# pedroand6/Voxel-Raytracer

Measured on AMD Instinct MI355X. Metric: Mrays/s at 1920×1080 primary rays; achieved HBM GB/s vs peak, higher is better.
Workload: dtype f32

## Files before the change

### voxel-raytracer_amd/__init__.py

```python
import ctypes as C
import os
import subprocess

import numpy as np

HERE = os.path.dirname(os.path.abspath(__file__))
CSRC = os.path.join(HERE, "csrc")
HIP_LIB = os.environ.get("VRT_HIP_LIB") or os.path.join(HERE, "libvrt_hip.so")
HOST_LIB = os.path.join(HERE, "libvrt_host.so")
TEST_LIB = os.path.join(HERE, "libvrt_hip_test.so")
OPT_RAY_TABLES, OPT_EMPTY_OCTANTS, OPT_DISPLAY_KERNEL, OPT_FULL_OPAQUE, OPT_HEAVY_TILES, OPT_MISS_TILES = 1, 2, 3, 4, 5, 6

MODE_PRIMARY, MODE_PRIMARY_SHADOW, MODE_FULL = 0, 1, 2
MODES = {"primary": MODE_PRIMARY, "primary_shadow": MODE_PRIMARY_SHADOW, "full": MODE_FULL}
ACCUM_JITTER = 1


class VrtError(RuntimeError):
    pass


def build(targets=("../libvrt_hip.so", "../libvrt_hip_test.so", "../libvrt_host.so")):
    subprocess.check_call(["make", "-j8", "-C", CSRC, *targets])

# ... 491 lines not shown

def miss_mask(texels, inv_proj, inv_view, cam_pos, width, height, voxel_scale=1.0, world_min=(-1023, -1023, -1023),
              world_max=(1024, 1024, 1024)):
    L = test_lib()
    L.vrt_test_miss_mask.argtypes = [C.c_void_p, C.c_size_t, C.POINTER(C.c_int32), C.POINTER(C.c_int32), C.c_float,
                                     C.POINTER(C.c_float), C.POINTER(C.c_float), C.POINTER(C.c_float), C.c_int, C.c_int,
                                     C.c_void_p, C.POINTER(C.c_int32)]
    t = np.ascontiguousarray(texels, np.uint8)
    ip = np.ascontiguousarray(inv_proj, np.float32).reshape(-1)
    iv = np.ascontiguousarray(inv_view, np.float32).reshape(-1)
    cp = np.zeros(4, np.float32)
    cp[:len(cam_pos)] = np.asarray(cam_pos, np.float32).reshape(-1)[:4]
    mask = np.zeros(((height + 7) // 8, (width + 7) // 8), np.uint8)
    stats = (C.c_int32 * 2)()
    r = L.vrt_test_miss_mask(t.ctypes.data if t.size else None, t.size, (C.c_int32 * 3)(*world_min), (C.c_int32 * 3)(*world_max),
                             float(voxel_scale), _fptr(ip), _fptr(iv), _fptr(cp), int(width), int(height), mask.ctypes.data, stats)
    if r < 0:
        raise VrtError(f"vrt_test_miss_mask failed ({r})")
    if r == 0:
        return None
    return mask, int(stats[0]), bool(stats[1])


def test_tile_order(tile_ticks, wave_slots, device=0):
    L = test_lib()
    t = np.ascontiguousarray(tile_ticks, np.uint32).reshape(-1)
    assert t.size % 4 == 0
    n = t.size // 4
    L.vrt_test_tile_order.argtypes = [C.c_int, C.c_void_p, C.c_uint32, C.c_uint32, C.c_void_p, C.c_void_p]
    order = np.zeros(n, np.uint32)
    split = np.zeros(1, np.uint32)
    r = L.vrt_test_tile_order(device, t.ctypes.data, n, wave_slots, order.ctypes.data, split.ctypes.data)
    if r:
        raise VrtError(f"vrt_test_tile_order failed ({r})")
    return order, int(split[0])



def tree_is_opaque(texels):
    L = test_lib()
    L.vrt_test_tree_is_opaque.argtypes = [C.c_void_p, C.c_size_t]
    t = np.ascontiguousarray(texels, np.uint8)
    r = L.vrt_test_tree_is_opaque(t.ctypes.data if t.size else None, t.size)
    if r < 0:
        raise VrtError(f"vrt_test_tree_is_opaque failed ({r})")
    return r == 1
# ... 484 lines not shown
```

### voxel-raytracer_amd/csrc/vrt_args.h

```cpp
#pragma once
#include <hip/hip_runtime.h>
#include <stdint.h>

namespace vrt {

struct F3 { float x, y, z; };
struct I3 { int x, y, z; };

constexpr int kMaxViews = 4;
constexpr int kGroupTiles = 4;
constexpr int kSplitParts = 8, kSplitMaxGroups = 64;
struct View {
    float inv_proj[16];
    float inv_view[16];
    float cam_pos[4];
    uint32_t *out_rgba;
    int2 *out_id;
    uint32_t eye0, eye1;
    uint32_t first_w0, first_w1, first_node, first_anode;
    int first_s, first_as, first_valid;
    const float *gen_x, *gen_y;
    float gen_z;
    uint32_t gen_fast;
    const uint8_t *miss;
    uint32_t miss_stamp;
};

struct ViewSet {
    View v[kMaxViews];
};

struct KArgs {
    int n_views;
    float voxel_scale;
    int wmin[3];
    int wmax[3];
    float global_light[4];
    float light_dir[3];
    float light_inv[3], light_push[3], light_dposf[3];
    int light_dpos[3];
    int shade_fast;
    int highlighted[3];
    int tex_dim;
    int width, height;
    int row0, n_rows, tile_rows, row_stride;
    int compact;
    uint32_t tiles_x_magic;
    int row_mode;
// ... 24 lines not shown
```

### voxel-raytracer_amd/csrc/vrt_common.hip.h

```cpp
#pragma once

#include "vrt_args.h"

namespace vrt {

#define VRT_DEV __device__ __forceinline__

VRT_DEV float fmin_c(float a, float b) { return b < a ? b : a; }
VRT_DEV float fmax_c(float a, float b) { return a < b ? b : a; }
VRT_DEV float dot3(F3 a, F3 b) { return (a.x * b.x + a.y * b.y) + a.z * b.z; }
VRT_DEV float len3(F3 a) { return __builtin_sqrtf(dot3(a, a)); }
VRT_DEV F3 scale3(F3 a, float s) { return F3{a.x * s, a.y * s, a.z * s}; }
VRT_DEV F3 add3(F3 a, F3 b) { return F3{a.x + b.x, a.y + b.y, a.z + b.z}; }
VRT_DEV F3 sub3(F3 a, F3 b) { return F3{a.x - b.x, a.y - b.y, a.z - b.z}; }
VRT_DEV F3 normalize3(F3 a) { return scale3(a, 1.0f / __builtin_sqrtf(dot3(a, a))); }

VRT_DEV float rcp_inrange(float x) {
    float y = __builtin_amdgcn_rcpf(x);
    y = __builtin_fmaf(__builtin_fmaf(-x, y, 1.0f), y, y);
    const float q = __builtin_fmaf(__builtin_fmaf(-x, y, 1.0f), y, y);
    return __builtin_fmaf(__builtin_fmaf(-x, q, 1.0f), y, q);
}
VRT_DEV float sqrt_inrange(float x) {
    const float s = __builtin_amdgcn_sqrtf(x);
// ... 106 lines not shown
    asm volatile("" : "+s"(p));
    return (LateView)p;
}

struct LateOut {
    uint32_t *out_rgba;
    int2 *out_id;
    int width, compact;
};
VRT_DEV LateOut late_out(LateArgs la, LateView lv) { return LateOut{lv->out_rgba, lv->out_id, la->width, la->compact}; }

VRT_DEV F3 shader_ray_dir(const KArgs &a, const View &vw, float fx, float fy) {
    float u = (fx / (float)a.width) * 2.0f - 1.0f;
    float v = (fy / (float)a.height) * 2.0f - 1.0f;
    float view[4];
    mat_vec(vw.inv_proj, u, v, -1.0f, 1.0f, view);
    if (__builtin_fabsf(view[3]) > 1e-6f) { float w = view[3]; view[0] = view[0] / w; view[1] = view[1] / w; view[2] = view[2] / w; view[3] = view[3] / w; }
    F3 vd = normalize3(F3{view[0], view[1], view[2]});
    float wd4[4];
    mat_vec(vw.inv_view, vd.x, vd.y, vd.z, 0.0f, wd4);
    return normalize3(F3{wd4[0], wd4[1], wd4[2]});
}

VRT_DEV F3 primary_ray_dir(const KArgs &a, const View &vw, int px, int py) {
    if (vw.gen_fast) {
        const F3 vd = normalize3_inrange(F3{vw.gen_x[px], vw.gen_y[py], vw.gen_z});
        float wd4[4];
        mat_vec(vw.inv_view, vd.x, vd.y, vd.z, 0.0f, wd4);
        const F3 d = normalize3_inrange(F3{wd4[0], wd4[1], wd4[2]});
        return scale3(d, rcp_inrange(sqrt_inrange(dot3(d, d))));
    }
    const F3 d = shader_ray_dir(a, vw, (float)px, (float)py);
    return scale3(d, 1.0f / __builtin_sqrtf(dot3(d, d)));
}

VRT_DEV float jitter_x(uint32_t k) { return (float)(__builtin_bitreverse32(k) >> 8) * 0x1p-24f; }
VRT_DEV float jitter_y(uint32_t k) {
    uint32_t y = 0u, v = 1u << 31;
    for (uint32_t i = k; i; i >>= 1, v ^= v >> 1)
        if (i & 1u) y ^= v;
    return (float)(y >> 8) * 0x1p-24f;
}

VRT_DEV F3 jittered_ray_dir(const KArgs &a, const View &vw, int px, int py, uint32_t sample) {
    const float fx = (float)px + jitter_x(sample), fy = (float)py + jitter_y(sample);
    const F3 d = shader_ray_dir(a, vw, fx, fy);
    return scale3(d, 1.0f / __builtin_sqrtf(dot3(d, d)));
}

struct LensRay { F3 o, dir; uint32_t eye0, eye1; };
VRT_DEV LensRay lens_ray(const KArgs &a, const View &vw, int px, int py, float jx, float jy, float aperture, float focus, float lx, float ly) {
    const float fx = (float)px + jx, fy = (float)py + jy;
    const F3 d = shader_ray_dir(a, vw, fx, fy);
    const F3 e{vw.cam_pos[0], vw.cam_pos[1], vw.cam_pos[2]};
    LensRay r;
    r.o = e; r.dir = d; r.eye0 = r.eye1 = 0u;
    const F3 R{vw.inv_view[0], vw.inv_view[1], vw.inv_view[2]}, U{vw.inv_view[4], vw.inv_view[5], vw.inv_view[6]},
             Z{vw.inv_view[8], vw.inv_view[9], vw.inv_view[10]};
    const float cosd = -dot3(d, Z);
    if (!(aperture == 0.0f || (lx == 0.0f && ly == 0.0f) || !(cosd > 0.0f))) {
        const float sx = aperture * lx, sy = aperture * ly;
        r.o = add3(add3(e, scale3(R, sx)), scale3(U, sy));
        const float t = focus / cosd;
        const F3 p = add3(e, scale3(d, t));
        r.dir = normalize3(sub3(p, r.o));
    }
    r.dir = scale3(r.dir, 1.0f / __builtin_sqrtf(dot3(r.dir, r.dir)));
    return r;
}

template <bool JIT, bool LENS>
VRT_DEV LensRay pixel_ray(const KArgs &a, const View &vw, int px, int py, uint32_t sample, const LensRay *lens) {
    if constexpr (LENS) return *lens;
    LensRay r;
    if constexpr (JIT) r.dir = jittered_ray_dir(a, vw, px, py, sample);
    else r.dir = primary_ray_dir(a, vw, px, py);
    r.o = F3{vw.cam_pos[0], vw.cam_pos[1], vw.cam_pos[2]};
    r.eye0 = vw.eye0;
    r.eye1 = vw.eye1;
    return r;
}

VRT_DEV void record_find(const KArgs &a, I3 p, uint32_t &w0, uint32_t &w1) {
    w0 = w1 = 0u;
    if (!in_world(a, p)) return;
    int mn[3] = {a.wmin[0], a.wmin[1], a.wmin[2]}, mx[3] = {a.wmax[0], a.wmax[1], a.wmax[2]};
    const int q[3] = {p.x, p.y, p.z};
    uint32_t rec = 0u;
    for (int i = 0; i < 16; ++i) {
        uint32_t ci = 0u;
#pragma unroll
        for (int k = 0; k < 3; ++k) {
            const int mid = mn[k] + ((mx[k] - mn[k]) >> 1);
            const bool hi = q[k] >= mid;
            if (hi) { ci |= 1u << (2 - k); mn[k] = mid; } else mx[k] = mid;
        }
        const uint2 r = a.nodes[rec];
        const uint32_t bit = 1u << ci;
        if (!(r.x & bit)) return;
        const uint32_t idx = r.y + (uint32_t)__builtin_popcount(r.x & 0xffu & (bit - 1u));
        if (idx >= a.n_records) return;
        if (r.x & (bit << 8)) { const uint2 l = a.nodes[idx]; w0 = l.x; w1 = l.y; return; }
        rec = idx;
    }
}

template <class T, class = void> struct host_light { static constexpr bool value = false; };
template <class T> struct host_light<T, decltype((void)T::kHostLight)> { static constexpr bool value = T::kHostLight; };
template <class T, class = void> struct miss_tiles { static constexpr bool value = false; };
template <class T> struct miss_tiles<T, decltype((void)T::kMissTiles)> { static constexpr bool value = T::kMissTiles; };

VRT_DEV bool miss_forward(F3 d) {
    return (d.x > 0.0f || d.x < -2e-8f) && (d.y > 0.0f || d.y < -2e-8f) && (d.z > 0.0f || d.z < -2e-8f);
}

constexpr uint32_t kSeedPlanes = 5, kSeedValid = 1u << 31;
struct Seed { F3 hp; uint32_t word; float iof; };

template <int MODE, class TRAV, bool JIT = false, bool LENS = false, bool MISS = false>
VRT_DEV void trace_pixel(const KArgs &a, const View &vw, const typename TRAV::Ctx &tc_, int px, int py, uint32_t &rgba, int2 &idd, LateOut &lo,
                         uint32_t *seed = nullptr, Seed *seed_regs = nullptr, uint32_t sample = 0u, const LensRay *lens = nullptr,
                         uint32_t miss_byte = 0u) {
    const float kPI = 3.14159265359f;
    const LensRay pr = pixel_ray<JIT, LENS>(a, vw, px, py, sample, lens);
    F3 ray_dir = pr.dir, ray_origin = pr.o;
    uint32_t eye0 = pr.eye0, eye1 = pr.eye1;

    int voxel_id = 0;
    int pixel_dist = a.wmax[0] - a.wmin[0];
    F3 gro = scale3(ray_origin, a.voxel_scale);
    Decoded tvd = decode_leaf(eye0, eye1);
    float start_iof = (tvd.p[0] > 0.0f && tvd.p[0] < 3.0f) ? tvd.p[0] : 1.0f;
    float medium_density = tvd.c[3] * 5.0f;
    float mc[3] = {1.0f, 1.0f, 1.0f};
    if (tvd.c[3] > 0.0f) { mc[0] = tvd.c[0]; mc[1] = tvd.c[1]; mc[2] = tvd.c[2]; }
    float fc[3] = {0.0f, 0.0f, 0.0f};
    const float sky[3] = {0.5f, 0.7f, 1.0f};

    Hit h;
    uint32_t seed_word = 0u;
    float seed_iof = 1.0f;
    const uint32_t eye_b = eye1 & 0xffu;
    const uint32_t iof_byte = (eye_b >= 1u && eye_b <= 254u) ? eye_b : 85u;
    bool hit = false;
    bool miss_tile = false;
    if constexpr (MISS) {
        static_assert((MODE == 0 || MODE == 1) && !JIT && !LENS && miss_tiles<TRAV>::value, "miss tiles: EYE85 primary rays only");
        asm volatile("" : "+v"(miss_byte) : "v"(ray_dir.x), "v"(ray_dir.y), "v"(ray_dir.z));
        miss_tile = miss_byte != vw.miss_stamp;
    }
    if (!(miss_tile && miss_forward(ray_dir))) hit = TRAV::march(a, tc_, gro, ray_dir, start_iof, iof_byte, h, &vw);
    constexpr bool kLate = MODE != 0;
    float l_gl[3] = {0.0f, 0.0f, 0.0f}, l_scale = 0.0f;
    F3 l_eye{0.0f, 0.0f, 0.0f}, l_light{0.0f, 0.0f, 0.0f};
    LightSetup l_ls{};
    int l_hl[3] = {0, 0, 0}, l_dim = 0, l_shade_fast = 0;
    if constexpr (kLate) {
        const LateArgs la = late_args();
        const LateView lv_ = late_view();
#pragma unroll
        for (int k = 0; k < 3; ++k) { l_gl[k] = la->global_light[k]; l_hl[k] = la->highlighted[k]; }
        l_scale = la->voxel_scale;
        l_dim = la->tex_dim;
        l_shade_fast = la->shade_fast;
        l_light = F3{la->light_dir[0], la->light_dir[1], la->light_dir[2]};
        if constexpr (MODE == 1 && host_light<TRAV>::value) {
            l_ls.dir = l_light;
            l_ls.inv = F3{la->light_inv[0], la->light_inv[1], la->light_inv[2]};
            l_ls.push = F3{la->light_push[0], la->light_push[1], la->light_push[2]};
            l_ls.dposf = F3{la->light_dposf[0], la->light_dposf[1], la->light_dposf[2]};
            l_ls.dpos = I3{la->light_dpos[0], la->light_dpos[1], la->light_dpos[2]};
        }
        if constexpr (!LENS) l_eye = F3{lv_->cam_pos[0], lv_->cam_pos[1], lv_->cam_pos[2]};
        lo = late_out(la, lv_);
    }
    const auto gl_ = [&](int k) { if constexpr (kLate) return l_gl[k]; else return a.global_light[k]; };
    const auto hl_ = [&](int k) { if constexpr (kLate) return l_hl[k]; else return a.highlighted[k]; };
    const float gl[3] = {gl_(0), gl_(1), gl_(2)};
    const auto scale_ = [&]() { if constexpr (kLate) return l_scale; else return a.voxel_scale; };
    const auto dim_ = [&]() { if constexpr (kLate) return l_dim; else return a.tex_dim; };
    const bool shade_fast = (kLate ? l_shade_fast : a.shade_fast) != 0;
    const auto eye_ = [&]() { if constexpr (kLate && !LENS) return l_eye; else return ray_origin; };
    const auto light_ = [&]() { if constexpr (kLate) return l_light; else return F3{a.light_dir[0], a.light_dir[1], a.light_dir[2]}; };
    float tc[3] = {gl[0], gl[1], gl[2]};
    if (!hit) {
#pragma unroll
        for (int k = 0; k < 3; ++k) fc[k] = fc[k] + gl[k] * sky[k] * tc[k] * 1.0f;
    } else {
        int naxis = h.axis;
        float nval = h.n;
        if (!(__builtin_fabsf(h.n) > 0.0f)) { naxis = 1; nval = 1.0f; }
        F3 hpw = h.point;
        if (scale_() != 1.0f) hpw = F3{h.point.x / scale_(), h.point.y / scale_(), h.point.z / scale_()};
        float dist_in_medium = 0.0f;
        if (medium_density > 0.0f) dist_in_medium = 0.0f + len3(sub3(hpw, scale3(eye_(), scale_()))) / scale_();
        Decoded hv = decode_leaf(h.h0, h.h1);
        if (hv.c[3] <= 0.0f) { hv.p[0] = 1.0f; hv.p[1] = 0.0f; hv.p[2] = 0.0f; }
        float sc[4] = {hv.c[0], hv.c[1], hv.c[2], hv.c[3]};
        uint32_t sc_bytes = h.h0 & 0x00ffffffu;
        if (__builtin_amdgcn_ballot_w64((h.h0 >> 24) == 0u) != 0ull) {
            const Decoded lv = decode_leaf(h.p0, h.p1);
            if (!(hv.c[3] > 0.0f)) { sc[0] = lv.c[0]; sc[1] = lv.c[1]; sc[2] = lv.c[2]; sc[3] = lv.c[3]; sc_bytes = h.p0 & 0x00ffffffu; }
        }
        if (dist_in_medium > 1e-6f && medium_density > 0.0f) {
            float kk = -medium_density * dist_in_medium;
#pragma unroll
            for (int k = 0; k < 3; ++k) tc[k] = tc[k] * det_expf(kk * (1.0f - mc[k]));
        }
        bool inverted = false;
        if (h.map.x == hl_(0) && h.map.y == hl_(1) && h.map.z == hl_(2)) {
// ... 25 lines not shown
            if (emission > 0.0f) {
#pragma unroll
                for (int k = 0; k < 3; ++k) fc[k] = fc[k] + tc[k] * sc[k] * emission * 1.0f;
            } else {
                int lit = 1;
                if constexpr (MODE == 1 && host_light<TRAV>::value) lit = TRAV::shadow(a, tc_, add3(h.point, scale3(normal, 2e-3f)), l_ls, h);
                else if constexpr (MODE == 1) lit = TRAV::shadow(a, tc_, add3(h.point, scale3(normal, 2e-3f)), light, h);
                if constexpr (MODE == 1) {
                    seed_word = kSeedValid | sc_bytes | ((uint32_t)naxis << 24) | (nval < 0.0f ? 1u << 26 : 0u) | (inverted ? 1u << 27 : 0u) |
                                (lit ? 1u << 28 : 0u);
                    const float prev_r = (h.p0 >> 24) != 0u ? refraction_of(h.p1) : 0.0f;
                    const float n1 = prev_r > 0.0f ? prev_r : 1.0f, n2 = hv.p[0] > 0.0f ? hv.p[0] : 1.0f;
                    seed_iof = flipped ? n2 : n1;
                }
#pragma unroll
                for (int k = 0; k < 3; ++k) {
                    float direct = gl[k] * (float)lit * ndotl;
                    const float num = direct * sc[k] * tc[k] * 1.0f;
                    fc[k] = fc[k] + (shade_fast ? div_pi_inrange(num) : num / kPI);
                }
            }
        }
    }
    rgba = unorm8(fc[0]) | (unorm8(fc[1]) << 8) | (unorm8(fc[2]) << 16) | (255u << 24);
    idd = make_int2(voxel_id, pixel_dist);
    if constexpr (MODE == 1) {
        if (seed_regs) { seed_regs->hp = h.point; seed_regs->word = seed_word; seed_regs->iof = seed_iof; }
        if (seed) {
            seed[3 * 64] = seed_word;
            if (seed_word) {
                seed[0] = __float_as_uint(h.point.x); seed[64] = __float_as_uint(h.point.y); seed[2 * 64] = __float_as_uint(h.point.z);
                seed[4 * 64] = __float_as_uint(seed_iof);
            }
        }
    }
}

namespace full {
template <class TRAV, bool JIT = false, bool LENS = false>
__device__ void trace_pixel_full(const KArgs &a, const View &vw, const typename TRAV::Ctx &tc_, int px, int py, uint32_t &rgba, int2 &idd, LateOut &lo,
                                 uint32_t sample = 0u, const LensRay *lens = nullptr);
template <class TRAV>
__device__ bool bounce_pixel(const KArgs &a, const typename TRAV::Ctx &tc_, int px, int py, Seed seed, uint32_t &rgba, uint32_t sample = 0u);
}

template <int MODE, class TRAV, int BLOCK, int WPE = 1, int SCHED = 0>
__global__ __launch_bounds__(BLOCK) __attribute__((amdgpu_waves_per_eu(WPE))) void trace_kernel(const KArgs a, const ViewSet vs) {
// ... 63 lines not shown
                if (seed.word & kSeedValid) {
                    seed.hp = F3{__uint_as_float(sp[0]), __uint_as_float(sp[64]), __uint_as_float(sp[2 * 64])};
                    seed.iof = __uint_as_float(sp[4 * 64]);
                }
                if (full::bounce_pixel<TRAV>(a, tc_, px, py, seed, rgba)) {
                    const LateArgs la = late_args();
                    const LateView lv_ = late_view();
                    lv_->out_rgba[(size_t)(la->compact ? j : py) * (size_t)la->width + (size_t)px] = rgba;
                }
            } else {
            if constexpr (MODE == 2)
                full::trace_pixel_full<TRAV>(a, vw, tc_, px, py, rgba, idd, lo);
            else if constexpr (MODE == 4)
                trace_pixel<1, TRAV>(a, vw, tc_, px, py, rgba, idd, lo, reinterpret_cast<uint32_t *>(a.defer_rec) + ((size_t)tile * kSeedPlanes) * 64 + lane);
            else if constexpr (MODE == 6) {
                Seed seed;
                seed.word = 0u;
                trace_pixel<1, TRAV>(a, vw, tc_, px, py, rgba, idd, lo, nullptr, &seed);
                uint32_t both;
                if (full::bounce_pixel<TRAV>(a, tc_, px, py, seed, both)) rgba = both;
            }
            else if constexpr ((MODE == 0 || MODE == 1) && miss_tiles<TRAV>::value) {
                uint32_t miss_byte = vw.miss_stamp;
                if (vw.miss) {
                    miss_byte = vw.miss[8u + (uint32_t)(py >> 3) * (uint32_t)((a.width + 7) >> 3) + (uint32_t)(px >> 3)];
                    if (*reinterpret_cast<const uint32_t *>(vw.miss) == vw.miss_stamp) miss_byte = vw.miss_stamp;
                }
                trace_pixel<MODE, TRAV, false, false, true>(a, vw, tc_, px, py, rgba, idd, lo, nullptr, nullptr, 0u, nullptr, miss_byte);
            }
            else trace_pixel<MODE, TRAV>(a, vw, tc_, px, py, rgba, idd, lo);
            if constexpr (MODE == 0) lo = LateOut{vw.out_rgba, vw.out_id, a.width, a.compact};
            size_t o = (size_t)(lo.compact ? j : py) * (size_t)lo.width + (size_t)px;
            if (lo.out_rgba) lo.out_rgba[o] = rgba;
            if (lo.out_id) lo.out_id[o] = idd;
            }
        }
        if constexpr (SCHED & 2) {
#ifndef VRT_EXP_STATS
            if (part_wave) { if (lane == 0) atomicMax(&a.tile_cost[tile], (uint32_t)(((__builtin_readcyclecounter() - t_begin) * 21ull) >> 4)); }
            else if (lane == 0) a.tile_cost[tile] = (uint32_t)(__builtin_readcyclecounter() - t_begin);
#endif
        }
    }
}

}
```

### voxel-raytracer_amd/csrc/vrt_dispatch.cpp

```cpp
#include "vrt_internal.h"

#include <algorithm>
#include <cmath>
#include <cstdio>
#include <new>

using namespace vrt_internal;
#include "vrt_launch.h"

namespace vrt_internal {

SchedState *sched_state(vrt_ctx *c, hipStream_t s, int width, int n_rows, int row0, int row_stride, int tile_rows, int mode,
                        uint32_t n_tiles, uint32_t n_groups) {
    uint64_t &tick = c->sched_tick;
    ++tick;
    for (SchedState &st : c->sched)
        if (st.stream == s && st.width == width && st.n_rows == n_rows && st.row0 == row0 && st.row_stride == row_stride &&
            st.tile_rows == tile_rows && st.mode == mode && st.n_tiles == n_tiles && st.n_groups == n_groups) {
            st.last_use = tick;
            return &st;
        }
    SchedState *slot = nullptr;
    if (c->sched.size() < kSchedMaxStates) {
        c->sched.emplace_back();
// ... 163 lines not shown
        m->ok = false;
        m->pending = true;
        m->last_use = ++c->miss_tick;
        return nullptr;
    }
    vrt_ctx::MissMask *m = hit;
    m->pending = false;
    m->last_use = ++c->miss_tick;
    vrt::miss::ViewParams vp;
    if (!t.fit_ok || !miss_view_params(w.inv_view, gro, t.fit, vp)) return nullptr;
    if (!m->built && hipEventCreateWithFlags(&m->built, hipEventDisableTiming) != hipSuccess) { m->built = nullptr; (void)hipGetLastError(); return nullptr; }
    if (!occupancy(c)) return nullptr;
    if (m->d_mask && (m->shared || m->stream != s) && hipDeviceSynchronize() != hipSuccess) return nullptr;
    const size_t bytes = 8 + (size_t)vp.tiles_x * (size_t)vp.tiles_y;
    if (bytes > m->capacity) {
        if (m->d_mask && hipDeviceSynchronize() != hipSuccess) return nullptr;
        uint32_t *fresh = nullptr;
        if (hipMalloc((void **)&fresh, bytes) != hipSuccess) { (void)hipGetLastError(); return nullptr; }
        (void)hipFree(m->d_mask);
        m->d_mask = fresh;
        m->capacity = bytes;
        m->stamp = 0;
    }
    if (m->stamp == 255u) m->stamp = 0u;
    m->stamp = (uint8_t)(m->stamp + 1u);
    if (m->stamp == 1u && hipMemsetAsync(m->d_mask, 0, m->capacity, s) != hipSuccess) { (void)hipGetLastError(); return nullptr; }
    if (vrt::launch::miss_mask(vp, c->occ.d_boxes, (uint32_t)c->occ.n_boxes, m->d_mask, m->stamp, s) != hipSuccess ||
        hipEventRecord(m->built, s) != hipSuccess) {
        (void)hipGetLastError();
        return nullptr;
    }
    m->stream = s;
    m->shared = false;
    m->ok = true;
    stamp = m->stamp;
    return reinterpret_cast<const uint8_t *>(m->d_mask);
}

int enqueue(vrt_ctx *c, int width, int height, int row0, int n_rows, int tile_rows, int row_stride, int compact,
            int mode, void *d_rgba, void *d_id, hipStream_t s, const vrt_view *views, int n_views, const AccumStep *acc) {
    if (!c->have_scene) return vrt_fail(c, VRT_E_STATE, "vrt_dispatch: no octree uploaded (call vrt_upload_octree first)");
    if (c->batch.open) return vrt_fail(c, VRT_E_STATE, "vrt_dispatch: a patch batch is open (call vrt_patch_end first)");
    if (!views && !c->have_camera) return vrt_fail(c, VRT_E_STATE, "vrt_dispatch: no camera set (call vrt_set_camera first)");
    if (n_views < 1 || n_views > vrt::kMaxViews) return vrt_fail(c, VRT_E_INVALID, "vrt_dispatch_views: 1 to 4 views per launch");
    if (mode != VRT_MODE_PRIMARY && mode != VRT_MODE_PRIMARY_SHADOW && mode != VRT_MODE_FULL)
        return vrt_fail(c, VRT_E_INVALID, "unknown mode");
    if (n_rows <= 0) return VRT_OK;
    {
        const int ra = ensure_analysis(c);
        if (ra) return ra;
// ... 15 lines not shown
    for (int i = 0; i < n_views; ++i) {
        vrt::View &w = vs.v[i];
        std::memcpy(w.inv_proj, views ? views[i].inv_projection : c->inv_proj, sizeof w.inv_proj);
        std::memcpy(w.inv_view, views ? views[i].inv_view : c->inv_view, sizeof w.inv_view);
        std::memcpy(w.cam_pos, views ? views[i].camera_pos : c->cam_pos, sizeof w.cam_pos);
        w.out_rgba = (uint32_t *)(views ? views[i].d_rgba8 : d_rgba);
        w.out_id = (int2 *)(views ? views[i].d_id_dist : d_id);
        int eye[3];
        for (int k = 0; k < 3; ++k) {
            const float g = floorf(w.cam_pos[k] * c->params.voxel_scale);
            eye[k] = g != g ? 0 : (g >= 2147483648.0f ? 2147483647 : (g < -2147483648.0f ? (-2147483647 - 1) : (int)g));
        }
        for (int k = 0; k < 3; ++k) eyes[i][k] = eye[k];
        vrt::eye_lookup(c->host_records, c->params.world_min, c->params.world_max, eye, w.eye0, w.eye1);
        vrt::FirstFind ff;
        w.first_valid = (c->wide_ok && vrt::first_find(c->wide, c->params.world_min, c->params.world_max, eye, vrt::v3::kAnchorShift, ff)) ? 1 : 0;
        if (w.first_valid) {
            w.first_w0 = ff.w0; w.first_w1 = ff.w1; w.first_node = ff.node; w.first_anode = ff.anode;
            w.first_s = ff.s; w.first_as = ff.as;
        }
        w.gen_x = w.gen_y = nullptr; w.gen_z = 0.0f; w.gen_fast = 0u;
        w.miss = nullptr;
        w.miss_stamp = 0u;
        tables[i] = nullptr;
        if (view_matrix_in_range(w.inv_view)) {
            if (const vrt_ctx::RayTable *t = ray_table(c, w.inv_proj, width, height)) {
                w.gen_x = t->d_tab; w.gen_y = t->d_tab + width; w.gen_z = t->z; w.gen_fast = 1u;
                tables[i] = t;
            }
        }
    }
    const bool lens = acc && acc->aperture > 0.0f;
    vrt::LensSel lsel;
    if (lens) {
        vrt::lens_select(c->host_records, c->wide_ok ? &c->wide : nullptr, c->params.world_min, c->params.world_max,
                         c->params.voxel_scale, vs.v[0].cam_pos, vs.v[0].inv_view, acc->aperture, lsel);
        if (!lsel.first_shared) vs.v[0].first_valid = 0;
    }
    if (v.trav == 4 && mode != VRT_MODE_FULL) {
        bool eye_in_medium = false;
        for (int i = 0; i < n_views; ++i) {
            const uint32_t b = vs.v[i].eye1 & 0xffu;
            eye_in_medium = eye_in_medium || (b >= 1u && b <= 254u && b != 85u);
        }
        if (lens) eye_in_medium = !lsel.no_medium;
        if (eye_in_medium) { v.trav = 3; v.wpe = 6; }
    }
    if (c->miss_tiles_on && !acc && v.trav == 4 && v.wpe == 7 && mode != VRT_MODE_FULL)
        for (int i = 0; i < n_views; ++i)
            if (tables[i]) vs.v[i].miss = miss_mask(c, vs.v[i], *tables[i], c->params.voxel_scale, s, vs.v[i].miss_stamp);
    a.voxel_scale = c->params.voxel_scale;
    for (int i = 0; i < 3; ++i) {
        a.wmin[i] = c->params.world_min[i];
        a.wmax[i] = c->params.world_max[i];
        a.light_dir[i] = c->params.light_dir[i];
        a.highlighted[i] = c->params.highlighted[i];
        const float d = a.light_dir[i];
        a.light_inv[i] = (fabsf(d) < 1e-8f) ? 1e20f : 1.0f / d;
        a.light_push[i] = (d > 0.0f ? 1.0f : (d < 0.0f ? -1.0f : 0.0f)) * 0.001f;
        a.light_dpos[i] = d > 0.0f ? 1 : 0;
        a.light_dposf[i] = d > 0.0f ? 1.0f : 0.0f;
    }
    for (int i = 0; i < 4; ++i) a.global_light[i] = c->params.global_light[i];
    a.shade_fast = 1;
    for (int i = 0; i < 3; ++i)
        if (!(fabsf(a.global_light[i]) <= 1073741824.0f) || !(fabsf(a.light_dir[i]) <= 1073741824.0f)) a.shade_fast = 0;
    a.tex_dim = (int)c->info.tex_dim;
    a.width = width;
    a.height = height;
    a.row0 = row0;
    a.n_rows = n_rows;
    a.tile_rows = tile_rows;
    a.row_stride = row_stride;
// ... 360 lines not shown

int vrt_set_option(vrt_ctx *c, int option, int value) {
    if (!c) return VRT_E_INVALID;
    switch (option) {
        case VRT_OPT_RAY_TABLES:
            if (value != 0 && value != 1) break;
            c->ray_tables_on = value != 0;
            return VRT_OK;
        case VRT_OPT_EMPTY_OCTANTS:
            if (value < 0 || value > 2) break;
            c->root0_only_on = value != 0;
            c->tight_root_on = value == 1;
            return VRT_OK;
        case VRT_OPT_FULL_OPAQUE:
            if (value != 0 && value != 1 && (value < 5 || value > 7)) break;
            c->two_pass_on = value != 0;
            c->two_pass_form = value;
            return VRT_OK;
        case VRT_OPT_HEAVY_TILES:
            if (value != 0 && value != 1) break;
            c->heavy_split_on = value != 0;
            return VRT_OK;
        case VRT_OPT_MISS_TILES:
            if (value != 0 && value != 1) break;
            c->miss_tiles_on = value != 0;
            return VRT_OK;
        case VRT_OPT_DISPLAY_KERNEL:
            if (value != 0 && value != 2 && value != 3) break;
            c->denoise_variant = value;
            return VRT_OK;
        default:
            return vrt_fail(c, VRT_E_INVALID, "vrt_set_option: unknown option");
    }
    return vrt_fail(c, VRT_E_INVALID, "vrt_set_option: value out of range");
}

int vrt_set_tile_order(vrt_ctx *c, int enable, const void *d_group_order, void *d_tile_cost) {
    if (!c) return VRT_E_INVALID;
    c->dbg_sched = enable != 0;
    c->dbg_group_order = enable ? (const uint32_t *)d_group_order : nullptr;
    c->dbg_tile_cost = enable ? (uint32_t *)d_tile_cost : nullptr;
    return VRT_OK;
}

long vrt_get_tile_order(vrt_ctx *c, void *stream, uint32_t *out, size_t cap) {
    if (!c) return VRT_E_INVALID;
    const SchedState *best = nullptr;
    for (const SchedState &st : c->sched)
// ... 11 lines not shown
```

### voxel-raytracer_amd/csrc/vrt_internal.h

```cpp
#pragma once
#include "../../include/vrt.h"

#include <hip/hip_runtime.h>

#include <cstring>
#include <string>
#include <vector>

#include "vrt_args.h"
#include "vrt_layout.h"
#include "vrt_miss.h"

struct Variant {
    int id;
    int trav;
    int wpe;
    int block() const { return trav >= 3 ? 64 : 256; }
};

inline constexpr Variant kVariants[] = {
    {0, 4, 7},
    {1, 1, 1},
    {4, 2, 1},
    {20, 3, 6},
// ... 66 lines not shown
    bool unit_internal = false;
    bool wide_ok = false;
    vrt::WideTree wide;
    uint2 *d_cells = nullptr;
    uint32_t *d_roots = nullptr;
    size_t cells_capacity = 0;
    int sched_period = 16;
    std::vector<SchedState> sched;
    uint64_t sched_tick = 0;
    bool order_lds_raised = false;
    struct RayTable {
        float inv_proj[16]{};
        int width = 0, height = 0;
        bool ok = false;
        float z = 0.0f;
        float *d_tab = nullptr;
        bool fit_ok = false;
        vrt::miss::TableFit fit{};
        size_t capacity = 0;
        uint64_t last_use = 0;
    };
    std::vector<RayTable> ray_tables;
    uint64_t ray_tick = 0;
    bool miss_tiles_on = true;
    struct Occupancy {
        bool built = false, ok = false;
        uint64_t tree_gen = 0;
        int wmin[3] = {0, 0, 0}, wmax[3] = {0, 0, 0};
        uint64_t seen_gen = ~0ull;
        int seen_wmin[3] = {0, 0, 0}, seen_wmax[3] = {0, 0, 0};
        uint64_t stable = 0;
        int *d_boxes = nullptr;
        size_t capacity = 0, n_boxes = 0;
    };
    Occupancy occ;
    struct MissMask {
        float inv_proj[16]{}, inv_view[16]{}, gro[3]{};
        int width = 0, height = 0;
        uint64_t tree_gen = 0;
        int wmin[3] = {0, 0, 0}, wmax[3] = {0, 0, 0};
        bool pending = false;
        bool ok = false;
        uint32_t *d_mask = nullptr;
        size_t capacity = 0;
        uint8_t stamp = 0;
        bool shared = false;
        hipStream_t stream = nullptr;
// ... 93 lines not shown
```

### voxel-raytracer_amd/csrc/vrt_launch.h

```cpp
#pragma once
#include "vrt_internal.h"
#include "vrt_query.h"
#include "vrt_accum.h"

namespace vrt {
namespace launch {

hipError_t trace_primary(const Variant &v, const KArgs &a, const ViewSet &vs, int grid, hipStream_t s, hipEvent_t ev0, hipEvent_t ev1);
hipError_t trace_shadow(const Variant &v, const KArgs &a, const ViewSet &vs, int grid, hipStream_t s, hipEvent_t ev0, hipEvent_t ev1);
hipError_t trace_full(const Variant &v, const KArgs &a, const ViewSet &vs, int grid, hipStream_t s, hipEvent_t ev0, hipEvent_t ev1);
hipError_t trace_full_opaque(const KArgs &a, const ViewSet &vs, int grid, int wpe, hipStream_t s, hipEvent_t ev0, hipEvent_t ev1);
hipError_t trace_full_two_pass(const KArgs &a, const ViewSet &vs, int grid, hipStream_t s, hipEvent_t ev0, hipEvent_t ev1);
hipError_t trace_full_pass1(const KArgs &a, const ViewSet &vs, int grid, hipStream_t s);
inline hipError_t trace(int mode, const Variant &v, const KArgs &a, const ViewSet &vs, int grid, hipStream_t s, hipEvent_t ev0, hipEvent_t ev1) {
    return mode == VRT_MODE_FULL ? trace_full(v, a, vs, grid, s, ev0, ev1)
                                 : (mode == VRT_MODE_PRIMARY ? trace_primary(v, a, vs, grid, s, ev0, ev1) : trace_shadow(v, a, vs, grid, s, ev0, ev1));
}

hipError_t tile_order(const uint32_t *d_cost, uint32_t n_groups, uint32_t *d_order, uint32_t wave_slots, bool raise_lds, size_t lds_ceiling, hipStream_t s);
hipError_t miss_mask(const miss::ViewParams &v, const int *d_boxes, uint32_t n, uint32_t *d_mask, uint8_t stamp, hipStream_t s);
hipError_t kernarg_probe(const KArgs &a, const ViewSet &vs, uint32_t *d_bad, hipStream_t s);

struct Denoise {
    const void *rgba, *id;
    void *out;
    int width, height;
    const uint32_t *group_order;
    uint32_t *tile_cost;
    int rows_path = 0;
};
void denoise_tiling(int width, int height, int &tiles_x, int &n_tiles);
hipError_t denoise(const Denoise &d, bool whole_groups, hipStream_t s);

hipError_t cast_rays(const KArgs &a, const query::RayArgs &q, hipStream_t s);
hipError_t find_voxels(const KArgs &a, const query::PointArgs &q, hipStream_t s);

hipError_t accum_primary(int mode, accum::Source src, const Variant &v, const KArgs &a, const ViewSet &vs, const accum::AdaptArgs &q,
                         bool adaptive, const accum::Lens &l, int grid, hipStream_t s);
hipError_t accum_opaque(accum::Source src, const KArgs &a, const ViewSet &vs, const accum::AdaptArgs &q, bool adaptive, const accum::Lens &l,
                        int grid, hipStream_t s);
hipError_t accum_full(accum::Source src, const Variant &v, const KArgs &a, const ViewSet &vs, const accum::AdaptArgs &q, bool adaptive,
                      const accum::Lens &l, int grid, hipStream_t s);
hipError_t accum_bounce(const KArgs &a, const ViewSet &vs, const accum::AdaptArgs &q, bool adaptive, int grid, hipStream_t s);
// ... 10 lines not shown
```

### voxel-raytracer_amd/csrc/vrt_launch_misc.hip

```cpp
#include <hip/hip_runtime.h>

#include "vrt_launch.h"
#include "vrt_sched.hip.h"
#include "vrt_denoise.hip.h"

namespace vrt {
namespace launch {

hipError_t tile_order(const uint32_t *d_cost, uint32_t n_groups, uint32_t *d_order, uint32_t wave_slots, bool raise_lds, size_t lds_ceiling, hipStream_t s) {
    const size_t lds = (size_t)n_groups * sizeof(uint32_t);
    if (raise_lds) {
        const hipError_t e = hipFuncSetAttribute(reinterpret_cast<const void *>(&tile_order_kernel), hipFuncAttributeMaxDynamicSharedMemorySize, (int)lds_ceiling);
        if (e != hipSuccess) return e;
    }
    hipLaunchKernelGGL(tile_order_kernel, dim3(1), dim3(1024), lds, s, (const uint4 *)d_cost, n_groups, d_order, wave_slots);
    return hipGetLastError();
}

constexpr uint32_t kMissLanes = 8;
__global__ __launch_bounds__(256) void miss_mask_kernel(const miss::ViewParams v, const miss::Box *boxes, uint32_t n, uint32_t *hdr,
                                                        uint32_t stamp) {
    uint8_t *mask = reinterpret_cast<uint8_t *>(hdr + 2);
    const uint32_t g = blockIdx.x * blockDim.x + threadIdx.x;
    const uint32_t i = g / kMissLanes, c = g % kMissLanes;
    if (i >= n) return;
    miss::Extent e = miss::project_corner(v, boxes[i], (int)c);
    for (int d = 1; d < (int)kMissLanes; d <<= 1) {
        miss::Extent o;
        o.lo_x = __shfl_xor(e.lo_x, d, kMissLanes); o.hi_x = __shfl_xor(e.hi_x, d, kMissLanes);
        o.lo_y = __shfl_xor(e.lo_y, d, kMissLanes); o.hi_y = __shfl_xor(e.hi_y, d, kMissLanes);
        o.behind = __shfl_xor(e.behind, d, kMissLanes); o.near = __shfl_xor(e.near, d, kMissLanes);
        e = miss::merge_extent(e, o);
    }
    int t[4];
    const int r = miss::extent_tiles(v, e, t);
    if (r == 2 && c == 0) hdr[0] = stamp;
    if (r == 1) {
        const uint32_t w = (uint32_t)(t[2] - t[0] + 1), cnt = w * (uint32_t)(t[3] - t[1] + 1);
        for (uint32_t k = c; k < cnt; k += kMissLanes) mask[(uint32_t)(t[1] + (int)(k / w)) * (uint32_t)v.tiles_x + (uint32_t)t[0] + k % w] = (uint8_t)stamp;
    }
}

hipError_t miss_mask(const miss::ViewParams &v, const int *d_boxes, uint32_t n, uint32_t *d_mask, uint8_t stamp, hipStream_t s) {
    const uint32_t blocks = n ? (uint32_t)(((uint64_t)n * kMissLanes + 255u) / 256u) : 1u;
    hipLaunchKernelGGL(miss_mask_kernel, dim3(blocks), dim3(256), 0, s, v, reinterpret_cast<const miss::Box *>(d_boxes), n, d_mask,
                       (uint32_t)stamp);
    return hipGetLastError();
}

hipError_t kernarg_probe(const KArgs &a, const ViewSet &vs, uint32_t *d_bad, hipStream_t s) {
    hipLaunchKernelGGL(kernarg_probe_kernel, dim3(1, kMaxViews), dim3(64), 0, s, a, vs, d_bad);
    return hipGetLastError();
}

void denoise_tiling(int width, int height, int &tiles_x, int &n_tiles) {
    tiles_x = (width + denoise::kTW - 1) / denoise::kTW;
    n_tiles = tiles_x * ((height + 15) / 16);
}

hipError_t denoise(const Denoise &d, bool whole_groups, hipStream_t s) {
    using namespace vrt::denoise;
    Args a;
    a.rgba = (const uint32_t *)d.rgba;
    a.id = (const int2 *)d.id;
    a.out = (uint32_t *)d.out;
    a.width = d.width;
    a.height = d.height;
    denoise_tiling(d.width, d.height, a.tiles_x, a.n_tiles);
    a.group_order = d.group_order;
// ... 15 lines not shown
```

Baseline: 55240.

## Precompute per-tile miss-forward state so whole-miss waves skip ray generation and traversal

Adds a second pass after the miss-mask build that marks 8x8 tiles where every primary ray both misses the occupancy boxes and points forward, encoded as stamp+1 (stamps now advance by two). In the tracing kernel, a wave whose tiles all carry that marker writes sky color and ids directly, skipping ray generation, miss_forward checks and traversal. Otherwise it passes preloaded gen_x/gen_y values into ray generation. This trades an extra small kernel launch and a wave ballot per pixel for removing per-ray work on fully empty sky regions. It relies on the forward kernel's ray directions matching the main kernel bit for bit.

```diff
diff --git a/voxel-raytracer_amd/__init__.py b/voxel-raytracer_amd/__init__.py
--- a/voxel-raytracer_amd/__init__.py
+++ b/voxel-raytracer_amd/__init__.py
@@ -537,6 +537,29 @@
     return mask, int(stats[0]), bool(stats[1])
 
 
+def miss_build(texels, inv_proj, inv_view, cam_pos, width, height, voxel_scale=1.0, world_min=(-1023, -1023, -1023),
+               world_max=(1024, 1024, 1024), device=0, dirs=True):
+    L = test_lib()
+    L.vrt_test_miss_build.argtypes = [C.c_int, C.c_void_p, C.c_size_t, C.POINTER(C.c_int32), C.POINTER(C.c_int32), C.c_float,
+                                      C.POINTER(C.c_float), C.POINTER(C.c_float), C.POINTER(C.c_float), C.c_int, C.c_int,
+                                      C.c_void_p, C.c_void_p]
+    t = np.ascontiguousarray(texels, np.uint8)
+    ip = np.ascontiguousarray(inv_proj, np.float32).reshape(-1)
+    iv = np.ascontiguousarray(inv_view, np.float32).reshape(-1)
+    cp = np.zeros(4, np.float32)
+    cp[:len(cam_pos)] = np.asarray(cam_pos, np.float32).reshape(-1)[:4]
+    state = np.zeros(((height + 7) // 8, (width + 7) // 8), np.uint8)
+    d = np.zeros((height, width, 3), np.float32) if dirs else None
+    r = L.vrt_test_miss_build(device, t.ctypes.data if t.size else None, t.size, (C.c_int32 * 3)(*world_min), (C.c_int32 * 3)(*world_max),
+                              float(voxel_scale), _fptr(ip), _fptr(iv), _fptr(cp), int(width), int(height), state.ctypes.data,
+                              d.ctypes.data if dirs else None)
+    if r < 0:
+        raise VrtError(f"vrt_test_miss_build failed ({r})")
+    if r == 0:
+        return None
+    return state, d
+
+
 def test_tile_order(tile_ticks, wave_slots, device=0):
     L = test_lib()
     t = np.ascontiguousarray(tile_ticks, np.uint32).reshape(-1)
diff --git a/voxel-raytracer_amd/csrc/vrt_args.h b/voxel-raytracer_amd/csrc/vrt_args.h
--- a/voxel-raytracer_amd/csrc/vrt_args.h
+++ b/voxel-raytracer_amd/csrc/vrt_args.h
@@ -24,6 +24,7 @@
     uint32_t gen_fast;
     const uint8_t *miss;
     uint32_t miss_stamp;
+    uint32_t miss_fwd;
 };
 
 struct ViewSet {
diff --git a/voxel-raytracer_amd/csrc/vrt_common.hip.h b/voxel-raytracer_amd/csrc/vrt_common.hip.h
--- a/voxel-raytracer_amd/csrc/vrt_common.hip.h
+++ b/voxel-raytracer_amd/csrc/vrt_common.hip.h
@@ -152,9 +152,12 @@
     return normalize3(F3{wd4[0], wd4[1], wd4[2]});
 }
 
-VRT_DEV F3 primary_ray_dir(const KArgs &a, const View &vw, int px, int py) {
+struct RayPre { float gx, gy; bool have; };
+VRT_DEV F3 primary_ray_dir(const KArgs &a, const View &vw, int px, int py, const RayPre *pre = nullptr) {
     if (vw.gen_fast) {
-        const F3 vd = normalize3_inrange(F3{vw.gen_x[px], vw.gen_y[py], vw.gen_z});
+        const bool have = pre && pre->have;
+        const float gx = have ? pre->gx : vw.gen_x[px], gy = have ? pre->gy : vw.gen_y[py];
+        const F3 vd = normalize3_inrange(F3{gx, gy, vw.gen_z});
         float wd4[4];
         mat_vec(vw.inv_view, vd.x, vd.y, vd.z, 0.0f, wd4);
         const F3 d = normalize3_inrange(F3{wd4[0], wd4[1], wd4[2]});
@@ -200,11 +203,11 @@
 }
 
 template <bool JIT, bool LENS>
-VRT_DEV LensRay pixel_ray(const KArgs &a, const View &vw, int px, int py, uint32_t sample, const LensRay *lens) {
+VRT_DEV LensRay pixel_ray(const KArgs &a, const View &vw, int px, int py, uint32_t sample, const LensRay *lens, const RayPre *pre = nullptr) {
     if constexpr (LENS) return *lens;
     LensRay r;
     if constexpr (JIT) r.dir = jittered_ray_dir(a, vw, px, py, sample);
-    else r.dir = primary_ray_dir(a, vw, px, py);
+    else r.dir = primary_ray_dir(a, vw, px, py, pre);
     r.o = F3{vw.cam_pos[0], vw.cam_pos[1], vw.cam_pos[2]};
     r.eye0 = vw.eye0;
     r.eye1 = vw.eye1;
@@ -244,15 +247,30 @@
     return (d.x > 0.0f || d.x < -2e-8f) && (d.y > 0.0f || d.y < -2e-8f) && (d.z > 0.0f || d.z < -2e-8f);
 }
 
+VRT_DEV void miss_shade(const float gl[3], float fc[3]) {
+    const float sky[3] = {0.5f, 0.7f, 1.0f};
+#pragma unroll
+    for (int k = 0; k < 3; ++k) fc[k] = fc[k] + gl[k] * sky[k] * gl[k] * 1.0f;
+}
+VRT_DEV uint32_t pack_rgba8(const float fc[3]) { return unorm8(fc[0]) | (unorm8(fc[1]) << 8) | (unorm8(fc[2]) << 16) | (255u << 24); }
+template <class ARGS>
+VRT_DEV void miss_pixel(const ARGS &a, uint32_t &rgba, int2 &idd) {
+    const float gl[3] = {a.global_light[0], a.global_light[1], a.global_light[2]};
+    float fc[3] = {0.0f, 0.0f, 0.0f};
+    miss_shade(gl, fc);
+    rgba = pack_rgba8(fc);
+    idd = make_int2(0, a.wmax[0] - a.wmin[0]);
+}
+
 constexpr uint32_t kSeedPlanes = 5, kSeedValid = 1u << 31;
 struct Seed { F3 hp; uint32_t word; float iof; };
 
 template <int MODE, class TRAV, bool JIT = false, bool LENS = false, bool MISS = false>
 VRT_DEV void trace_pixel(const KArgs &a, const View &vw, const typename TRAV::Ctx &tc_, int px, int py, uint32_t &rgba, int2 &idd, LateOut &lo,
                          uint32_t *seed = nullptr, Seed *seed_regs = nullptr, uint32_t sample = 0u, const LensRay *lens = nullptr,
-                         uint32_t miss_byte = 0u) {
+                         uint32_t miss_byte = 0u, const RayPre *pre = nullptr) {
     const float kPI = 3.14159265359f;
-    const LensRay pr = pixel_ray<JIT, LENS>(a, vw, px, py, sample, lens);
+    const LensRay pr = pixel_ray<JIT, LENS>(a, vw, px, py, sample, lens, pre);
     F3 ray_dir = pr.dir, ray_origin = pr.o;
     uint32_t eye0 = pr.eye0, eye1 = pr.eye1;
 
@@ -265,7 +283,6 @@
     float mc[3] = {1.0f, 1.0f, 1.0f};
     if (tvd.c[3] > 0.0f) { mc[0] = tvd.c[0]; mc[1] = tvd.c[1]; mc[2] = tvd.c[2]; }
     float fc[3] = {0.0f, 0.0f, 0.0f};
-    const float sky[3] = {0.5f, 0.7f, 1.0f};
 
     Hit h;
     uint32_t seed_word = 0u;
@@ -276,7 +293,6 @@
     bool miss_tile = false;
     if constexpr (MISS) {
         static_assert((MODE == 0 || MODE == 1) && !JIT && !LENS && miss_tiles<TRAV>::value, "miss tiles: EYE85 primary rays only");
-        asm volatile("" : "+v"(miss_byte) : "v"(ray_dir.x), "v"(ray_dir.y), "v"(ray_dir.z));
         miss_tile = miss_byte != vw.miss_stamp;
     }
     if (!(miss_tile && miss_forward(ray_dir))) hit = TRAV::march(a, tc_, gro, ray_dir, start_iof, iof_byte, h, &vw);
@@ -314,8 +330,7 @@
     const auto light_ = [&]() { if constexpr (kLate) return l_light; else return F3{a.light_dir[0], a.light_dir[1], a.light_dir[2]}; };
     float tc[3] = {gl[0], gl[1], gl[2]};
     if (!hit) {
-#pragma unroll
-        for (int k = 0; k < 3; ++k) fc[k] = fc[k] + gl[k] * sky[k] * tc[k] * 1.0f;
+        miss_shade(gl, fc);
     } else {
         int naxis = h.axis;
         float nval = h.n;
@@ -387,7 +402,7 @@
             }
         }
     }
-    rgba = unorm8(fc[0]) | (unorm8(fc[1]) << 8) | (unorm8(fc[2]) << 16) | (255u << 24);
+    rgba = pack_rgba8(fc);
     idd = make_int2(voxel_id, pixel_dist);
     if constexpr (MODE == 1) {
         if (seed_regs) { seed_regs->hp = h.point; seed_regs->word = seed_word; seed_regs->iof = seed_iof; }
@@ -497,11 +512,25 @@
             }
             else if constexpr ((MODE == 0 || MODE == 1) && miss_tiles<TRAV>::value) {
                 uint32_t miss_byte = vw.miss_stamp;
+                RayPre pre{0.0f, 0.0f, vw.miss != nullptr};
+                bool fast = false;
                 if (vw.miss) {
                     miss_byte = vw.miss[8u + (uint32_t)(py >> 3) * (uint32_t)((a.width + 7) >> 3) + (uint32_t)(px >> 3)];
+                    pre.gx = vw.gen_x[px];
+                    pre.gy = vw.gen_y[py];
                     if (*reinterpret_cast<const uint32_t *>(vw.miss) == vw.miss_stamp) miss_byte = vw.miss_stamp;
+                    fast = __builtin_amdgcn_ballot_w64(miss_byte != vw.miss_fwd) == 0ull;
                 }
-                trace_pixel<MODE, TRAV, false, false, true>(a, vw, tc_, px, py, rgba, idd, lo, nullptr, nullptr, 0u, nullptr, miss_byte);
+                if (fast) {
+                    if constexpr (MODE == 0) miss_pixel(a, rgba, idd);
+                    else {
+                        const LateArgs la = late_args();
+                        miss_pixel(*la, rgba, idd);
+                        lo = late_out(la, late_view());
+                    }
+                } else {
+                    trace_pixel<MODE, TRAV, false, false, true>(a, vw, tc_, px, py, rgba, idd, lo, nullptr, nullptr, 0u, nullptr, miss_byte, &pre);
+                }
             }
             else trace_pixel<MODE, TRAV>(a, vw, tc_, px, py, rgba, idd, lo);
             if constexpr (MODE == 0) lo = LateOut{vw.out_rgba, vw.out_id, a.width, a.compact};
diff --git a/voxel-raytracer_amd/csrc/vrt_dispatch.cpp b/voxel-raytracer_amd/csrc/vrt_dispatch.cpp
--- a/voxel-raytracer_amd/csrc/vrt_dispatch.cpp
+++ b/voxel-raytracer_amd/csrc/vrt_dispatch.cpp
@@ -209,10 +209,9 @@
         m->capacity = bytes;
         m->stamp = 0;
     }
-    if (m->stamp == 255u) m->stamp = 0u;
-    m->stamp = (uint8_t)(m->stamp + 1u);
+    m->stamp = (m->stamp == 0u || m->stamp >= 253u) ? (uint8_t)1u : (uint8_t)(m->stamp + 2u);
     if (m->stamp == 1u && hipMemsetAsync(m->d_mask, 0, m->capacity, s) != hipSuccess) { (void)hipGetLastError(); return nullptr; }
-    if (vrt::launch::miss_mask(vp, c->occ.d_boxes, (uint32_t)c->occ.n_boxes, m->d_mask, m->stamp, s) != hipSuccess ||
+    if (vrt::launch::miss_mask(vp, w, c->occ.d_boxes, (uint32_t)c->occ.n_boxes, m->d_mask, m->stamp, s) != hipSuccess ||
         hipEventRecord(m->built, s) != hipSuccess) {
         (void)hipGetLastError();
         return nullptr;
@@ -274,6 +273,7 @@
         w.gen_x = w.gen_y = nullptr; w.gen_z = 0.0f; w.gen_fast = 0u;
         w.miss = nullptr;
         w.miss_stamp = 0u;
+        w.miss_fwd = 0x100u;
         tables[i] = nullptr;
         if (view_matrix_in_range(w.inv_view)) {
             if (const vrt_ctx::RayTable *t = ray_table(c, w.inv_proj, width, height)) {
@@ -298,9 +298,12 @@
         if (lens) eye_in_medium = !lsel.no_medium;
         if (eye_in_medium) { v.trav = 3; v.wpe = 6; }
     }
-    if (c->miss_tiles_on && !acc && v.trav == 4 && v.wpe == 7 && mode != VRT_MODE_FULL)
+    if (c->miss_tiles && !acc && v.trav == 4 && v.wpe == 7 && mode != VRT_MODE_FULL)
         for (int i = 0; i < n_views; ++i)
-            if (tables[i]) vs.v[i].miss = miss_mask(c, vs.v[i], *tables[i], c->params.voxel_scale, s, vs.v[i].miss_stamp);
+            if (tables[i]) {
+                vs.v[i].miss = miss_mask(c, vs.v[i], *tables[i], c->params.voxel_scale, s, vs.v[i].miss_stamp);
+                if (vs.v[i].miss && c->miss_tiles == 2) vs.v[i].miss_fwd = vs.v[i].miss_stamp + 1u;
+            }
     a.voxel_scale = c->params.voxel_scale;
     for (int i = 0; i < 3; ++i) {
         a.wmin[i] = c->params.world_min[i];
@@ -707,8 +710,8 @@
             c->heavy_split_on = value != 0;
             return VRT_OK;
         case VRT_OPT_MISS_TILES:
-            if (value != 0 && value != 1) break;
-            c->miss_tiles_on = value != 0;
+            if (value < 0 || value > 2) break;
+            c->miss_tiles = value;
             return VRT_OK;
         case VRT_OPT_DISPLAY_KERNEL:
             if (value != 0 && value != 2 && value != 3) break;
diff --git a/voxel-raytracer_amd/csrc/vrt_internal.h b/voxel-raytracer_amd/csrc/vrt_internal.h
--- a/voxel-raytracer_amd/csrc/vrt_internal.h
+++ b/voxel-raytracer_amd/csrc/vrt_internal.h
@@ -112,7 +112,7 @@
     };
     std::vector<RayTable> ray_tables;
     uint64_t ray_tick = 0;
-    bool miss_tiles_on = true;
+    int miss_tiles = 2;
     struct Occupancy {
         bool built = false, ok = false;
         uint64_t tree_gen = 0;
diff --git a/voxel-raytracer_amd/csrc/vrt_launch.h b/voxel-raytracer_amd/csrc/vrt_launch.h
--- a/voxel-raytracer_amd/csrc/vrt_launch.h
+++ b/voxel-raytracer_amd/csrc/vrt_launch.h
@@ -18,7 +18,7 @@
 }
 
 hipError_t tile_order(const uint32_t *d_cost, uint32_t n_groups, uint32_t *d_order, uint32_t wave_slots, bool raise_lds, size_t lds_ceiling, hipStream_t s);
-hipError_t miss_mask(const miss::ViewParams &v, const int *d_boxes, uint32_t n, uint32_t *d_mask, uint8_t stamp, hipStream_t s);
+hipError_t miss_mask(const miss::ViewParams &v, const View &vw, const int *d_boxes, uint32_t n, uint32_t *d_mask, uint8_t stamp, hipStream_t s);
 hipError_t kernarg_probe(const KArgs &a, const ViewSet &vs, uint32_t *d_bad, hipStream_t s);
 
 struct Denoise {
diff --git a/voxel-raytracer_amd/csrc/vrt_launch_misc.hip b/voxel-raytracer_amd/csrc/vrt_launch_misc.hip
--- a/voxel-raytracer_amd/csrc/vrt_launch_misc.hip
+++ b/voxel-raytracer_amd/csrc/vrt_launch_misc.hip
@@ -2,6 +2,7 @@
 
 #include "vrt_launch.h"
 #include "vrt_sched.hip.h"
+#include "vrt_miss.hip.h"
 #include "vrt_denoise.hip.h"
 
 namespace vrt {
@@ -17,34 +18,14 @@
     return hipGetLastError();
 }
 
-constexpr uint32_t kMissLanes = 8;
-__global__ __launch_bounds__(256) void miss_mask_kernel(const miss::ViewParams v, const miss::Box *boxes, uint32_t n, uint32_t *hdr,
-                                                        uint32_t stamp) {
-    uint8_t *mask = reinterpret_cast<uint8_t *>(hdr + 2);
-    const uint32_t g = blockIdx.x * blockDim.x + threadIdx.x;
-    const uint32_t i = g / kMissLanes, c = g % kMissLanes;
-    if (i >= n) return;
-    miss::Extent e = miss::project_corner(v, boxes[i], (int)c);
-    for (int d = 1; d < (int)kMissLanes; d <<= 1) {
-        miss::Extent o;
-        o.lo_x = __shfl_xor(e.lo_x, d, kMissLanes); o.hi_x = __shfl_xor(e.hi_x, d, kMissLanes);
-        o.lo_y = __shfl_xor(e.lo_y, d, kMissLanes); o.hi_y = __shfl_xor(e.hi_y, d, kMissLanes);
-        o.behind = __shfl_xor(e.behind, d, kMissLanes); o.near = __shfl_xor(e.near, d, kMissLanes);
-        e = miss::merge_extent(e, o);
-    }
-    int t[4];
-    const int r = miss::extent_tiles(v, e, t);
-    if (r == 2 && c == 0) hdr[0] = stamp;
-    if (r == 1) {
-        const uint32_t w = (uint32_t)(t[2] - t[0] + 1), cnt = w * (uint32_t)(t[3] - t[1] + 1);
-        for (uint32_t k = c; k < cnt; k += kMissLanes) mask[(uint32_t)(t[1] + (int)(k / w)) * (uint32_t)v.tiles_x + (uint32_t)t[0] + k % w] = (uint8_t)stamp;
-    }
-}
-
-hipError_t miss_mask(const miss::ViewParams &v, const int *d_boxes, uint32_t n, uint32_t *d_mask, uint8_t stamp, hipStream_t s) {
+hipError_t miss_mask(const miss::ViewParams &v, const View &vw, const int *d_boxes, uint32_t n, uint32_t *d_mask, uint8_t stamp, hipStream_t s) {
     const uint32_t blocks = n ? (uint32_t)(((uint64_t)n * kMissLanes + 255u) / 256u) : 1u;
     hipLaunchKernelGGL(miss_mask_kernel, dim3(blocks), dim3(256), 0, s, v, reinterpret_cast<const miss::Box *>(d_boxes), n, d_mask,
                        (uint32_t)stamp);
+    const hipError_t e = hipGetLastError();
+    if (e != hipSuccess) return e;
+    const uint32_t tiles = (uint32_t)v.tiles_x * (uint32_t)v.tiles_y;
+    hipLaunchKernelGGL(miss_forward_kernel, dim3((tiles + 3u) / 4u), dim3(256), 0, s, vw, v.width, v.height, d_mask, (uint32_t)stamp);
     return hipGetLastError();
 }
 
diff --git a/voxel-raytracer_amd/csrc/vrt_miss.hip.h b/voxel-raytracer_amd/csrc/vrt_miss.hip.h
--- /dev/null
+++ b/voxel-raytracer_amd/csrc/vrt_miss.hip.h
@@ -0,0 +1,48 @@
+#pragma once
+
+#include "vrt_common.hip.h"
+#include "vrt_miss.h"
+
+namespace vrt {
+
+constexpr uint32_t kMissLanes = 8;
+__global__ __launch_bounds__(256) void miss_mask_kernel(const miss::ViewParams v, const miss::Box *boxes, uint32_t n, uint32_t *hdr,
+                                                        uint32_t stamp) {
+    uint8_t *mask = reinterpret_cast<uint8_t *>(hdr + 2);
+    const uint32_t g = blockIdx.x * blockDim.x + threadIdx.x;
+    const uint32_t i = g / kMissLanes, c = g % kMissLanes;
+    if (i >= n) return;
+    miss::Extent e = miss::project_corner(v, boxes[i], (int)c);
+    for (int d = 1; d < (int)kMissLanes; d <<= 1) {
+        miss::Extent o;
+        o.lo_x = __shfl_xor(e.lo_x, d, kMissLanes); o.hi_x = __shfl_xor(e.hi_x, d, kMissLanes);
+        o.lo_y = __shfl_xor(e.lo_y, d, kMissLanes); o.hi_y = __shfl_xor(e.hi_y, d, kMissLanes);
+        o.behind = __shfl_xor(e.behind, d, kMissLanes); o.near = __shfl_xor(e.near, d, kMissLanes);
+        e = miss::merge_extent(e, o);
+    }
+    int t[4];
+    const int r = miss::extent_tiles(v, e, t);
+    if (r == 2 && c == 0) hdr[0] = stamp;
+    if (r == 1) {
+        const uint32_t w = (uint32_t)(t[2] - t[0] + 1), cnt = w * (uint32_t)(t[3] - t[1] + 1);
+        for (uint32_t k = c; k < cnt; k += kMissLanes) mask[(uint32_t)(t[1] + (int)(k / w)) * (uint32_t)v.tiles_x + (uint32_t)t[0] + k % w] = (uint8_t)stamp;
+    }
+}
+
+__global__ __launch_bounds__(256) void miss_forward_kernel(const View vw, int width, int height, uint32_t *hdr, uint32_t stamp) {
+    uint8_t *mask = reinterpret_cast<uint8_t *>(hdr + 2);
+    const int tiles_x = (width + miss::kTile - 1) / miss::kTile, tiles_y = (height + miss::kTile - 1) / miss::kTile;
+    const int tile = (int)(blockIdx.x * (blockDim.x / 64u) + (threadIdx.x >> 6)), lane = (int)(threadIdx.x & 63u);
+    if (tile >= tiles_x * tiles_y) return;
+    if (mask[tile] == (uint8_t)stamp) return;
+    const int px = (tile % tiles_x) * miss::kTile + lane % miss::kTile, py = (tile / tiles_x) * miss::kTile + lane / miss::kTile;
+    bool fails = false;
+    if (px < width && py < height) {
+        KArgs a;
+        a.width = width; a.height = height;
+        fails = !miss_forward(primary_ray_dir(a, vw, px, py));
+    }
+    if (__builtin_amdgcn_ballot_w64(fails) == 0ull && lane == 0) mask[tile] = (uint8_t)(stamp + 1u);
+}
+
+}
```

New measurement: 55380 (median of 4 runs). No clear change (+0.2%).
